# ElijahHyndman/PAPTeam_OpticalFlow

Measured on AMD Instinct MI355X. Metric: Mpix/s per frame-pair (fixed SOR iters) at 1920x1080; max-abs d(u,v) vs ref, higher is better.
Workload: dtype f64

## Files before the change

include/papof.h:

```cpp
#ifndef PAPOF_H
#define PAPOF_H

#include <stddef.h>

#ifdef __cplusplus
extern "C" {
#endif

#define PAPOF_VERSION 115

enum {
    PAPOF_OK = 0,
    PAPOF_EINVAL = -1,
    PAPOF_ENODEVICE = -2,
    PAPOF_ENOMEM = -3,
    PAPOF_EDEVICE = -4,
    PAPOF_ETIMEOUT = -5
};

enum {
    PAPOF_SOR_EXACT = 0,
    PAPOF_SOR_REDBLACK = 1,
    PAPOF_SOR_JACOBI = 2
};
// ... 443 lines not shown

int papof_deblur_tensor(papof_handle* h, int n_frames, int height, int width, int c, const papof_tensor* frames,
                        const papof_tensor* flow_fw, const papof_tensor* flow_bw, int n_samples, const double* offsets,
                        const double* weights, int radius, int iters, int use_check, double alpha1, double alpha2,
                        const papof_tensor* out, const papof_tensor* support, void* workspace, long long workspace_bytes,
                        void* stream);
long long papof_deblur_workspace(int n_frames, int height, int width, int c, int radius);

enum { PAPOF_ROWS_MAX_KNOTS = 4096 };
int papof_warp_rows_tensor(papof_handle* h, int n_frames, int height, int width, int c, const papof_tensor* frames,
                           const papof_tensor* matrices, int n_knots, int iters, const papof_tensor* out,
                           const papof_tensor* valid, void* stream);

int papof_last_host_times(papof_handle* h, double out[3]);

int papof_test_sor_strips(papof_handle* h, int height, int width, int n_sor, int split_band, int reps, int delay_us,
                          long long* mismatches, int* bands);

int papof_test_poison(papof_handle* h, unsigned long long pattern, size_t* bytes);

#ifdef __cplusplus
}
#endif
#endif
```

papteam_opticalflow_amd/capi.py:

```python
import ctypes
import os

import numpy as np

_HERE = os.path.dirname(os.path.abspath(__file__))
LIB_PATH = os.path.join(_HERE, "csrc", "libpapof.so")

SOR_EXACT, SOR_REDBLACK, SOR_JACOBI = 0, 1, 2
N_TIMERS = 10

_D = ctypes.POINTER(ctypes.c_double)
_I = ctypes.POINTER(ctypes.c_int)
c_int, c_double, c_void_p = ctypes.c_int, ctypes.c_double, ctypes.c_void_p


class Params(ctypes.Structure):
    _fields_ = [("alpha", c_double), ("ratio", c_double), ("n_outer", c_int), ("n_outer_per_level", c_int),
                ("n_inner", c_int), ("n_sor", c_int), ("n_sor_per_level", c_int), ("omega", c_double),
                ("sor_mode", c_int), ("phase_timing", c_int), ("interpolation", c_int), ("noise_model", c_int)]


DTYPE_U8, DTYPE_F32, DTYPE_F64 = 0, 1, 2
DTYPE_U16 = 3
MOTION_SIMILARITY, MOTION_AFFINE = 0, 1
# ... 17 lines not shown

SYMBOLS = [
    "papof_version", "papof_default_params", "papof_strerror", "papof_last_error", "papof_timing_key",
    "papof_device_count", "papof_create", "papof_destroy", "papof_coarse2fine_flow", "papof_flow",
    "papof_flow_device", "papof_dev_alloc", "papof_dev_free", "papof_dev_upload", "papof_dev_download",
    "papof_stream", "papof_stage_pyramid", "papof_stage_gaussian", "papof_stage_resize_ratio",
    "papof_stage_resize_wh", "papof_stage_im2feature", "papof_stage_warpFL", "papof_stage_getDxs",
    "papof_stage_linear_system", "papof_stage_laplacian", "papof_stage_sor", "papof_stage_smoothflow",
    "papof_stage_bicubic_warp", "papof_bench_sor", "papof_flow_u8", "papof_flow_device_u8", "papof_seq_reset",
    "papof_seq_push", "papof_seq_push_u8", "papof_seq_push_device", "papof_tiles_grid", "papof_tiles_rect",
    "papof_tiles_halo_message", "papof_tiles_unique_id", "papof_tiles_create", "papof_tiles_create_local",
    "papof_tiles_flow_device", "papof_tiles_stats", "papof_tiles_destroy", "papof_flow_quantize16",
    "papof_flow_dequantize16", "papof_flow_to_bgr", "papof_set_stream_overlap", "papof_sor_plan", "papof_last_sor_stats", "papof_test_sor_strips",
    "papof_pyramid_levels_for_min_width", "papof_stage_smoothflow_ex", "papof_stage_est_gaussian_mixture",
    "papof_stage_bicubic_warp_ex", "papof_tiles_comm_info", "papof_host_alloc", "papof_host_free",
    "papof_last_sor_solves", "papof_bands_plan", "papof_lap_guard_stats", "papof_last_host_times",
    "papof_flow_batch", "papof_flow_batch_u8", "papof_batch_stats", "papof_flow_batch_tensor", "papof_flow_batch_tensor_fb",
    "papof_fb_check_tensor", "papof_track_tensor", "papof_interp_tensor", "papof_flow_batch_tensor_init",
    "papof_flow_batch_tensor_fb_init", "papof_motion_fit_tensor", "papof_motion_workspace", "papof_warp_affine_tensor",
    "papof_temporal_filter_tensor", "papof_fill_holes_tensor", "papof_fill_workspace", "papof_propagate_tensor",
    "papof_temporal_consistency_tensor", "papof_consistency_workspace", "papof_splat_tensor", "papof_splat_workspace",
    "papof_interp_splat_tensor", "papof_refine_flow_tensor", "papof_refine_workspace", "papof_refine_tables",
    "papof_super_resolve_tensor", "papof_sr_workspace", "papof_match_tensor", "papof_match_workspace",
    "papof_match_hier_tensor", "papof_match_hier_workspace", "papof_match_recentre_tensor", "papof_match_recentre_workspace",
    "papof_match_densify_tensor", "papof_motion_blur_tensor", "papof_decimate_tensor", "papof_upsample_flow_tensor",
    "papof_upsample_tables", "papof_mosaic_tensor", "papof_mosaic_blend_tensor", "papof_mosaic_overlap_tensor", "papof_sor_tiny_shape",
    "papof_homography_workspace", "papof_homography_fit_tensor", "papof_warp_projective_tensor",
    "papof_mosaic_projective_tensor", "papof_mosaic_overlap_projective_tensor",
    "papof_mosaic_ray_tensor", "papof_mosaic_overlap_ray_tensor",
    "papof_bundle_workspace", "papof_bundle_sums_tensor",
    "papof_mesh_workspace", "papof_mesh_motion_tensor", "papof_warp_mesh_tensor",
# ... 84 lines not shown
    L.papof_stage_smoothflow_ex.argtypes = [c_void_p, _D, _D, _D, _D, _D, c_int, c_int, c_int, c_double, c_int, c_int,
                                            c_int, c_double, c_int, c_int, c_int, _D]
    L.papof_stage_est_gaussian_mixture.argtypes = [c_void_p, _D, _D, c_int, c_int, c_int, _D]
    L.papof_stage_bicubic_warp_ex.argtypes = [c_void_p, _D, _D, _D, _D, c_int, c_int, c_int, c_int, _D]
    L.papof_pyramid_levels_for_min_width.argtypes = [c_int, c_double, c_int, ctypes.POINTER(c_int)]
    L.papof_sor_tiny_shape.argtypes = [c_int, c_int, ctypes.POINTER(c_int), ctypes.POINTER(c_int)]
    L.papof_host_alloc.argtypes = [ctypes.c_size_t, ctypes.POINTER(c_void_p)]
    L.papof_host_free.argtypes = [c_void_p]
    L.papof_sor_plan.argtypes = [c_void_p, c_int, c_int, c_int, c_int, ctypes.POINTER(c_int), ctypes.POINTER(c_int)]
    L.papof_last_sor_stats.argtypes = [c_void_p, ctypes.POINTER(c_int), ctypes.POINTER(ctypes.c_double)]
    L.papof_last_sor_solves.argtypes = [c_void_p, c_int, ctypes.POINTER(c_int), ctypes.POINTER(c_int),
                                        ctypes.POINTER(ctypes.c_double)]
    L.papof_lap_guard_stats.argtypes = [c_void_p, ctypes.POINTER(c_int)]
    L.papof_last_host_times.argtypes = [c_void_p, ctypes.POINTER(c_double)]
    L.papof_batch_stats.argtypes = [c_void_p, ctypes.POINTER(ctypes.c_longlong)]
    for fn in (L.papof_flow_batch, L.papof_flow_batch_u8):
        fn.argtypes = [c_void_p, c_int, c_int, c_void_p, c_int, c_int, c_int, c_int, c_void_p, c_void_p, c_void_p, c_void_p, _D]
        fn.restype = c_int
    _T = ctypes.POINTER(PapofTensor)
    L.papof_flow_batch_tensor.argtypes = [c_void_p, c_int, c_int, _T, _T, c_int, c_int, c_int, c_int, PP, _T, _T, c_void_p, _D]
    L.papof_flow_batch_tensor.restype = c_int
    L.papof_flow_batch_tensor_fb.argtypes = [c_void_p, c_int, c_int, _T, _T, c_int, c_int, c_int, c_int, PP, _T, _T, _T, _T, _T,
                                             c_double, c_double, c_void_p, _D]
    L.papof_flow_batch_tensor_fb.restype = c_int
    L.papof_flow_batch_tensor_init.argtypes = [c_void_p, c_int, c_int, _T, _T, c_int, c_int, c_int, c_int, PP, _T, _T, _T,
                                               c_void_p, _D]
    L.papof_flow_batch_tensor_init.restype = c_int
    L.papof_flow_batch_tensor_fb_init.argtypes = [c_void_p, c_int, c_int, _T, _T, c_int, c_int, c_int, c_int, PP, _T, _T, _T,
                                                  _T, _T, _T, _T, c_double, c_double, c_void_p, _D]
    L.papof_flow_batch_tensor_fb_init.restype = c_int
# ... 587 lines not shown
        t = np.zeros(N_TIMERS)
        PP = ctypes.c_void_p * len(fr)
        fp = PP(*[f.ctypes.data for f in fr])
        OP = ctypes.c_void_p * n_pairs
        ox, oy, ow = (OP(*[o[i].ctypes.data for o in out]) for i in range(3))
        pp = ctypes.byref(params) if params is not None else None
        fn = self.L.papof_flow_batch_u8 if u8 else self.L.papof_flow_batch
        _chk(fn(self.h, n_pairs, 1 if sequence else 0, fp, h, w, c, int(levels), pp, ox, oy, ow, _p(t)), "papof_flow_batch")
        return out, t

    def batch_stats(self):
        out = (ctypes.c_longlong * 4)()
        _chk(self.L.papof_batch_stats(self.h, out), "papof_batch_stats")
        return dict(chains=out[0], chain_pairs=out[1], singles=out[2], reruns=out[3])

    def last_host_times(self):
        out = (c_double * 3)()
        _chk(self.L.papof_last_host_times(self.h, out), "papof_last_host_times")
        return out[0], out[1]

    def lap_guard_stats(self):
        out = (c_int * 4)()
        _chk(self.L.papof_lap_guard_stats(self.h, out), "papof_lap_guard_stats")
        return dict(reruns=out[0], exact_calls=out[1], exact_next=bool(out[2]), guard_on=bool(out[3]))

    def test_sor_strips(self, h, w, n_sor, split_band, reps=3, delay_us=0):
        mm, nb = ctypes.c_longlong(0), c_int(0)
        _chk(self.L.papof_test_sor_strips(self.h, h, w, n_sor, split_band, reps, delay_us, ctypes.byref(mm),
                                          ctypes.byref(nb)), "papof_test_sor_strips")
        return mm.value, nb.value

    def test_poison(self, pattern=0x7FF8DEAD7FF8DEAD):
        n = ctypes.c_size_t(0)
        _chk(self.L.papof_test_poison(self.h, pattern, ctypes.byref(n)), "papof_test_poison")
# ... 179 lines not shown
```

papteam_opticalflow_amd/csrc/api.hip:

```cpp
#include <algorithm>
#include <chrono>
#include <cmath>
#include <cstdio>
#include <cstdlib>
#include <cstring>
#include <mutex>
#include <random>
#include <thread>

#include "common.h"
#include "flow_internal.h"

namespace papof {

namespace {
thread_local std::string g_last_error;
}

void set_last_error(const char* what, hipError_t e, const char* file, int line) {
    char buf[512];
    std::snprintf(buf, sizeof buf, "%s failed: %s (%s:%d)", what, hipGetErrorString(e), file, line);
    g_last_error = buf;
}
const char* last_error() { return g_last_error.c_str(); }
// ... 302 lines not shown

struct LevelSolve {
    SolveBuffers& B;
    const double *f1 = nullptr, *f2 = nullptr;
    double* warp = nullptr;
    int H = 0, W = 0, fc = 0;
    double alpha = 0, omega = 0;
    int n_outer = 0, n_inner = 0, n_sor = 0, mode = PAPOF_SOR_EXACT;
    const double* im1s_ready = nullptr;
    bool final_warp = true;
    const SolveCounters* counters = nullptr;
    double *out_u = nullptr, *out_v = nullptr;
    bool fold_warp = false;
    LapGuard* lg = nullptr;
    int level = 0;
};

static int marked_solve(papof_handle* h, PhaseClock& clk, unsigned* prog, SorPlanes& SP, const LevelSolve& s) {
    h->sor_mark = [](void* c, int on) {
        static_cast<PhaseClock*>(c)->phase(on ? PAPOF_T_PHASE5_SOR : PAPOF_T_PHASE6_UPDATE);
    };
    h->sor_mark_ctx = &clk;
    h->sor_prog_next = prog;
    const int rc = sor_solve(h, SP, s.H, s.W, s.alpha, s.omega, s.n_sor, s.mode);
    h->sor_prog_next = nullptr;
    h->sor_mark = nullptr;
    h->sor_mark_ctx = nullptr;
    return rc;
}

int smooth_flow(papof_handle* h, const LevelSolve& s, PhaseClock& clk, double*& u, double*& v, double*& ua, double*& va) {
    SolveBuffers& B = s.B;
    const Taps g = smooth5_taps();
    int solve_idx = 0;
    const bool tiny = s.mode == PAPOF_SOR_EXACT && B.sp_tiny.phi && sor_tiny_fits(h, s.H, s.W, s.n_sor);
    SorPlanes& SP = tiny ? B.sp_tiny : B.sp;
    const double* im1s = s.im1s_ready;
    if (!im1s) {
        clk.phase(PAPOF_T_PHASE1_GENERATE);
        PAPOF_TRY(filter_hv(h, s.f1, B.im1s, B.tmp, s.H, s.W, s.fc, g, g));
        im1s = B.im1s;
    }
    const char* const fused_sw = std::getenv("PAPOF_FUSED_SYSTEM");
    const bool fused_env = !(fused_sw && fused_sw[0] == '0');
    const bool fused_system = fused_env && s.fold_warp && s.n_inner == 1 && !B.gm && (s.fc == 5 || s.fc == 3) &&
                              !(s.lg && s.lg->guard()) && !(s.lg && s.lg->on && lap_one_block_level(s.H, s.W));
    for (int count = 0; count < s.n_outer; count++) {
        clk.phase(fused_system ? kTimerFused : (int)PAPOF_T_PHASE1_GENERATE);
        if (fused_system)
            PAPOF_TRY(flow_system(h, s.f1, s.f2, u, v, im1s, s.H, s.W, s.fc, s.alpha, s.omega, SP,
                                  s.lg && count > 0 ? s.lg->wit(s.lg->slot - 1) : nullptr));
        else if (s.fold_warp)
            PAPOF_TRY(warp_smooth_blend(h, s.f1, s.f2, u, v, im1s, B.blend, B.imdt, s.H, s.W, s.fc,
                                        s.lg && count > 0 && !B.gm ? s.lg->wit(s.lg->slot - 1) : nullptr,
                                        B.phi));
        else
            PAPOF_TRY(smooth_hv_blend(h, s.warp, im1s, B.blend, B.imdt, s.H, s.W, s.fc));
        for (int hh = 0; hh < s.n_inner; hh++) {
            const SorPlanes* prev = hh == 0 ? nullptr : &SP;
            if ((count == 0 && !s.fold_warp) || hh > 0) {
                clk.phase(PAPOF_T_PHASE2_DERIVATIVES);
                PAPOF_TRY(compute_phi(h, u, v, prev, B.phi, s.H, s.W));
            }
            if (!fused_system) clk.phase(PAPOF_T_PHASE4_LINEARSYSTEM);
            if (!fused_system)
                PAPOF_TRY(assemble_system(h, B.blend, B.imdt, B.phi, u, v, s.H, s.W, s.fc, s.alpha, s.omega, SP, nullptr, nullptr,
                                          prev, nullptr, B.gm, s.lg ? s.lg->guard() : nullptr));
            PAPOF_TRY(marked_solve(h, clk, s.counters ? s.counters->solve(h, s.level, (size_t)solve_idx) : nullptr, SP, s));
            solve_idx++;
        }
        double* const phi_next = count + 1 < s.n_outer && !s.fold_warp ? B.phi : nullptr;
        const bool rewarp = !s.fold_warp && !B.bgx && (s.final_warp || count + 1 < s.n_outer || B.gm);
        const bool wit_later = s.fold_warp && count + 1 < s.n_outer;
        const bool wit_small = s.fold_warp && !wit_later && lap_one_block_level(s.H, s.W);
        unsigned* const wit = s.lg && !B.gm && !B.bgx && !wit_later && !wit_small ? s.lg->wit(s.lg->slot) : nullptr;
        const bool to_caller = s.out_u && s.out_v && count + 1 == s.n_outer;
        PAPOF_TRY(update_warp_phi(h, SP, u, v, to_caller ? s.out_u : ua, to_caller ? s.out_v : va, s.f1, s.f2, s.warp, phi_next,
                                  s.H, s.W, s.fc, rewarp, 0, -1, wit));
        if (to_caller) {
            u = s.out_u;
            v = s.out_v;
        } else {
            std::swap(u, ua);
            std::swap(v, va);
        }
        if (B.bgx)
            PAPOF_TRY(bicubic_warp(h, s.f1, s.f2, B.bgx, B.bgy, B.bgxy, u, v, s.warp, s.H, s.W, s.fc, nullptr, true, true));
        if (s.lg && s.lg->on && !B.gm && wit_small && s.lg->wit(s.lg->slot))
            PAPOF_TRY(lap_small_check(h, s.f1, s.f2, u, v, s.H, s.W, s.fc, s.lg->wit(s.lg->slot)));
        if (s.lg && s.lg->on && !B.gm) {
            s.lg->slot_level.push_back(s.level);
            s.lg->slot_channels.push_back(s.fc);
            s.lg->slot++;
            if (s.lg->exact) {
// ... 43 lines not shown
    LapGuard* lg;
    const papof_tensor* init;
    CallPlan cp;
    int slot1 = 0;
    double *tmp_a = nullptr, *tmp_b = nullptr;
    std::vector<double*> F1, F2, S1;
    double *prep_tmp = nullptr, *warp = nullptr;
    double *u = nullptr, *v = nullptr, *u2 = nullptr, *v2 = nullptr;
    SolveBuffers B;
    bool exact = false;
    SolveCounters counters;
    bool overlap = false;
    bool hostio = false;
    hipStream_t main_stream = nullptr, prep = nullptr;
    PhaseClock clk, pclk, total;
};

static void keep_seq(const FlowPass& S, int slot) {
    S.h->seq = {.valid = true, .h = S.H, .w = S.W, .c = S.C, .levels = S.cp.levels, .slot = slot, .ratio = S.cp.ratio,
                .arena_base = S.h->arena.base};
}

static void start_clocks(FlowPass& S) {
    papof_handle* h = S.h;
    S.clk = S.pclk = S.total = PhaseClock{h, true};
    S.clk.only_sor = S.pclk.only_sor = (!h->phase_events && S.P.phase_timing == 0) || S.P.phase_timing == 2;
    h->sor_launches = 0;
    h->sor_log.clear();
    S.clk.stamps = true;
    h->stamps_used = 0;
    h->next_stamp = nullptr;
    h->stamp_stream = h->stream;
    S.total.phase(PAPOF_T_TOTAL);
}

static int carve_pyramids(FlowPass& S) {
    Arena& A = S.h->arena;
    for (Level& l : S.cp.L) {
        double* slot[2];
        slot[0] = A.f64((size_t)l.w * l.h * S.C);
        slot[1] = A.f64((size_t)l.w * l.h * S.C);
        l.p1 = slot[S.slot1];
        l.p2 = slot[S.slot1 ^ 1];
// ... 139 lines not shown
    S.v = S.u + np;
    S.v2 = S.u2 + np;
    if (B.bgx) PAPOF_TRY(central3_planes(h, f2, B.bgx, B.bgy, B.bgxy, lh, lw, fc));
    if (coarsest && !S.init) return PAPOF_OK;
    if (B.bgx)
        PAPOF_TRY(bicubic_warp(h, f1, f2, B.bgx, B.bgy, B.bgxy, S.u, S.v, S.warp, lh, lw, fc, nullptr, true, false));
    else if (!fold_warp)
        PAPOF_TRY(warp_bilinear(h, f1, f2, S.u, S.v, S.warp, lh, lw, fc));
    return PAPOF_OK;
}

static int solve_levels(FlowPass& S) {
    papof_handle* h = S.h;
    const CallPlan& cp = S.cp;
    LapGuard* const lg = S.lg;
    if (lg && lg->guard())
        PAPOF_HIP(hipMemcpyAsync(lg->lap, h->lap_init_dev, 8 * sizeof(double), hipMemcpyDeviceToDevice, S.main_stream));
    int pw = 0, ph = 0;
    for (int k = cp.levels - 1; k >= 0; k--) {
        const int lw = cp.L[k].w, lh = cp.L[k].h;
        S.clk.phase(-1);
        if (S.overlap) PAPOF_HIP(hipStreamWaitEvent(S.main_stream, h->sync_events[k], 0));
        S.clk.phase(PAPOF_T_ALLOCATION);
        const bool tiny_k = S.exact && sor_tiny_fits(h, lh, lw, cp.n_sor[k]);
        if (!tiny_k) PAPOF_TRY(sor_bind(h, S.B.sp, lh, lw, cp.n_sor[k]));
        const LevelSolve s{.B = S.B, .f1 = S.F1[k], .f2 = S.F2[k], .warp = S.warp, .H = lh, .W = lw, .fc = cp.fc,
                           .alpha = S.P.alpha, .omega = S.P.omega, .n_outer = cp.n_outer[k], .n_inner = S.P.n_inner,
                           .n_sor = cp.n_sor[k], .mode = S.P.sor_mode, .im1s_ready = S.S1[k], .final_warp = false,
                           .counters = S.exact ? &S.counters : nullptr, .out_u = k == 0 ? S.d_vx : nullptr,
                           .out_v = k == 0 ? S.d_vy : nullptr, .fold_warp = !S.B.bgx && !S.B.gm, .lg = lg, .level = k};
        PAPOF_TRY(enter_level(S, k, pw, ph, s.fold_warp));
        if (!tiny_k) PAPOF_TRY(sor_reset_planes(h, S.B.sp));
        PAPOF_TRY(smooth_flow(h, s, S.clk, S.u, S.v, S.u2, S.v2));
        pw = lw;
        ph = lh;
    }
    return PAPOF_OK;
}

static int final_warp(FlowPass& S) {
    papof_handle* h = S.h;
    papof_handle::HostIO& io = h->hostio;
    const int H = S.H, W = S.W, C = S.C;
    const size_t np0 = (size_t)H * W;
    const Level& l0 = S.cp.L[0];
    S.clk.phase(PAPOF_T_POSTPROCESSING);
    if (S.hostio && io.early_out && S.u == S.d_vx && S.v == S.d_vy) {
// ... 49 lines not shown
    }
    {
        const double f = tm[kTimerFused];
        tm[PAPOF_T_PHASE1_GENERATE] += 0.51 * f;
        tm[PAPOF_T_PHASE2_DERIVATIVES] += 0.02 * f;
        tm[PAPOF_T_PHASE3_PSIDATA] += 0.14 * f;
        tm[PAPOF_T_PHASE4_LINEARSYSTEM] += f - 0.51 * f - 0.02 * f - 0.14 * f;
    }
}

int flow_pass(papof_handle* h, const FrameIn& fa, const FrameIn& fb, SeqOp op, int H, int W, int C, int levels,
              const papof_params& P, double* d_vx, double* d_vy, double* d_warp, double* timing, LapGuard* lg,
              const papof_tensor* init = nullptr) {
    const double t_entry = wall();
    FlowPass S{h, fa, fb, op, H, W, C, P, d_vx, d_vy, d_warp, lg, init};
    PAPOF_TRY(call_plan(H, W, C, levels, P, S.cp));
    const size_t need = arena_bytes_for(H, W, C, levels, S.cp.n_sor_max, P.ratio);
    if (op == kSeqNext && !seq_matches(h, H, W, C, levels, S.cp.ratio, need)) {
        g_last_error = "sequence push does not continue the primed sequence (shape, levels, ratio or arena changed)";
        return PAPOF_EINVAL;
    }
    S.slot1 = op == kSeqNext ? h->seq.slot : 0;
    h->seq.valid = false;
    PAPOF_TRY(ensure_arena(h, need));
    h->arena.off = 0;
    h->arena.overflow = false;
    h->events_used = 0;
    double tm[PAPOF_N_TIMERS + 1];
    std::memset(tm, 0, sizeof tm);
    start_clocks(S);
// ... 974 lines not shown
}

int papof_lap_guard_stats(papof_handle* h, int out[4]) {
    if (!h || !out) return PAPOF_EINVAL;
    out[0] = h->lap_reruns;
    out[1] = h->lap_exact_calls;
    out[2] = h->lap_exact ? 1 : 0;
    out[3] = h->lap_guard ? 1 : 0;
    return PAPOF_OK;
}

int papof_last_host_times(papof_handle* h, double out[3]) {
    if (!h || !out) return PAPOF_EINVAL;
    out[0] = h->host_enqueue_sec;
    out[1] = h->host_wait_sec;
    out[2] = 0.0;
    return PAPOF_OK;
}

int papof_last_sor_solves(papof_handle* h, int cap, int* n, int* info, double* sec) {
    if (!h || !n) return PAPOF_EINVAL;
    *n = (int)h->sor_log.size();
    for (int i = 0; i < *n && i < cap; i++) {
        const papof_handle::SorSolveLog& e = h->sor_log[i];
        if (info) {
            int* o = info + (size_t)i * 6;
            o[0] = e.H;
            o[1] = e.W;
            o[2] = e.n_sor;
            o[3] = e.kind;
            o[4] = e.depth;
// ... 229 lines not shown
```

papteam_opticalflow_amd/csrc/common.h:

```cpp
#pragma once
#include <cstdlib>

#include <hip/hip_runtime.h>

#include <algorithm>
#include <cmath>
#include <cstddef>
#include <cstdint>
#include <initializer_list>
#include <string>
#include <vector>

#include "../../include/papof.h"

namespace papof {

constexpr int kLanes = 64;
constexpr int kMaxFsize = 8;

struct Rect {
    int x0, y0, x1, y1;
    __host__ __device__ bool empty() const { return x1 <= x0 || y1 <= y0; }
    __host__ __device__ int w() const { return x1 - x0; }
    __host__ __device__ int h() const { return y1 - y0; }
// ... 155 lines not shown
    hipEvent_t entry_event = nullptr;
    unsigned* init_flag_dev = nullptr;
    bool use_dpp = false;
    int sor_depth = 0;
    unsigned long long* sor_dbg = nullptr;
    void (*sor_mark)(void*, int) = nullptr;
    void* sor_mark_ctx = nullptr;
    int sor_fuse = 0;
    int sor_group = 0;
    int rb_depth = 0;
    int rb_shape = 0;
    int sor_tiny = 1;
    int sor_resident = 0;
    int sor_skip_dead = 1;
    unsigned* sor_prog_next = nullptr;
    int sor_launches = 0;
    struct SorSolveLog {
        int H, W, n_sor, kind, depth, launches;
        double sec;
    };
    std::vector<SorSolveLog> sor_log;
    hipStream_t prep_stream = nullptr;
    unsigned* lap_flags_dev = nullptr;
    unsigned* lap_flags_host = nullptr;
    double* lap_dev = nullptr;
    double* lap_init_dev = nullptr;
    double* lap_scratch_dev = nullptr;
    bool lap_guard = true;
    bool lap_exact = false;
    unsigned lap_epoch = 0;
    int lap_reruns = 0, lap_exact_calls = 0;
    long long batch_chains = 0, batch_chain_pairs = 0, batch_singles = 0, batch_reruns = 0;
    double host_enqueue_sec = 0.0, host_wait_sec = 0.0;
    struct HostIO {
        bool active = false;
        const void *im1 = nullptr, *im2 = nullptr;
        size_t nb_in = 0;
        double *vx = nullptr, *vy = nullptr, *warp = nullptr;
        size_t nb_flow = 0, nb_img = 0;
        bool early_out = false;
        bool out_issued = false;
    } hostio;
    hipStream_t copy_stream = nullptr;
    std::vector<hipEvent_t> copy_events;
    std::vector<hipEvent_t> sync_events;
    bool overlap_prep = true;
    unsigned long long* stamps_dev = nullptr;
// ... 72 lines not shown
                   int W, int planes, const Rect* rc = nullptr);
int smooth_hv_blend(papof_handle* h, const double* warp, const double* im1s, double* blend, double* imdt, int H,
                    int W, int planes, int row0 = 0, int row1 = -1);
int warp_smooth_blend(papof_handle* h, const double* im1, const double* im2, const double* u, const double* v,
                      const double* im1s, double* blend, double* imdt, int H, int W, int planes, unsigned* wit = nullptr,
                      double* phi_out = nullptr);
int compute_phi(papof_handle* h, const double* u, const double* v, const SorPlanes* prev, double* phi, int H, int W,
                const Rect* rc = nullptr);
int assemble_system(papof_handle* h, const double* blend, const double* imdt, const double* phi, const double* u,
                    const double* v, int H, int W, int planes, double alpha, double omega, const SorPlanes& out,
                    double* opt_imdx2, double* opt_imdy2, const SorPlanes* prev, const Rect* rc = nullptr,
                    const double* gm = nullptr, const double* lap = nullptr);
int flow_system(papof_handle* h, const double* im1, const double* im2, const double* u, const double* v, const double* im1s,
                int H, int W, int planes, double alpha, double omega, const SorPlanes& out, unsigned* wit = nullptr,
                int row0 = 0, int row1 = -1,
                int batch = 1, const BatchK* bk = nullptr);
int lap_scratch_doubles();
int lap_rows_check(papof_handle* h, const double* im1, const double* im2, const double* u, const double* v, int H, int W,
                   int C, int r0, int r1, unsigned* wit, unsigned* val, unsigned mark);
bool lap_one_block_level(int H, int W);
int lap_small_check(papof_handle* h, const double* im1, const double* im2, const double* u, const double* v, int H, int W,
                    int C, unsigned* wit, int batch = 1, const BatchK* bk = nullptr);
int est_laplacian_noise(papof_handle* h, const double* im1, const double* im2, const double* u, const double* v, int H,
                        int W, int C, double* lap, double* scratch);
int gm_scratch_doubles();
int est_gaussian_mixture(papof_handle* h, const double* im1, const double* im2, int H, int W, int C, double* gm,
                         double* scratch);
int laplacian(papof_handle* h, const double* in, const double* weight, double* out, int H, int W);
int bicubic_warp(papof_handle* h, const double* im1, const double* im2, const double* gx, const double* gy,
                 const double* gxy, const double* vx, const double* vy, double* out_hwc, int H, int W, int C,
                 const Rect* rc = nullptr, bool planar_out = false, bool clamp = true, int batch = 1, const BatchK* bk = nullptr);
// ... 33 lines not shown
};
int sor_solve_bands(papof_handle* h, const SorPlanes& sp, int H, int W, double alpha, double omega, int n_sor,
                    unsigned* prog, int b0, int b1, const SorSplit* split = nullptr);
int sor_bind_plain(papof_handle* h, SorPlanes& sp, int H, int W, int n_sor);
constexpr size_t kTinyMaxCells = 8192;
bool sor_tiny_fits(const papof_handle* h, int H, int W, int n_sor);
bool sor_tiny_shape(int H, int W, int* cells_per_tile, int* waves);
int sor_alloc_tiny_planes(Arena& A, size_t cells, SorPlanes& sp);
size_t sor_counters_words(int H, int W, int n_sor);
int sor_counters_ensure(papof_handle* h, size_t words);
unsigned* sor_counters_clear(papof_handle* h, size_t offset_words, size_t words);
int sor_alloc_planes(Arena& A, int H, int W, int mode, int n_sor_cap, SorPlanes& sp);
int sor_bind(papof_handle* h, SorPlanes& sp, int H, int W, int n_sor);
int sor_group_size(const papof_handle* h, int H, int W, int n_sor);
int sor_reset_planes(papof_handle* h, const SorPlanes& sp);
int sor_reset_planes_batch(papof_handle* h, const SorPlanes& sp, int batch, size_t stride);
int sor_probe_dpp(papof_handle* h);

}
```

papteam_opticalflow_amd/csrc/kernels.hip:

```cpp
#include "common.h"
#include "sampler.h"

#include <cmath>
#include <type_traits>

namespace papof {

namespace {

constexpr int BX = 64, BY = 4;

constexpr int tiles_of(int n, int t) { return (n + t - 1) / t; }
inline dim3 grid2d(int W, int H, int planes = 1) { return dim3(tiles_of(W, BX), tiles_of(H, BY), planes); }
inline Rect region(const Rect* rc, int W, int H) { return rc ? *rc : Rect{0, 0, W, H}; }
inline dim3 grid2d(const Rect& r, int planes = 1) { return grid2d(r.x1 - r.x0, r.y1 - r.y0, planes); }

__device__ __forceinline__ void stamp_now(unsigned long long* s) {
    if (s && (blockIdx.x | blockIdx.y | blockIdx.z | threadIdx.x | threadIdx.y) == 0u) *s = __builtin_amdgcn_s_memrealtime();
}
__global__ void k_stamp(unsigned long long* s) { stamp_now(s); }

__host__ __device__ __forceinline__ int clampi(int x, int n) {
    x = x < 0 ? 0 : x;
    return x > n - 1 ? n - 1 : x;
// ... 989 lines not shown
    double* q[6];
};
typedef double tap_pair __attribute__((ext_vector_type(2), aligned(8)));
__device__ __forceinline__ double plane_ld(const double* plane, unsigned byte_off) {
    return *reinterpret_cast<const double*>(reinterpret_cast<const char*>(plane) + byte_off);
}
__device__ __forceinline__ tap_pair plane_ld2(const double* plane, unsigned byte_off) {
    return *reinterpret_cast<const tap_pair*>(reinterpret_cast<const char*>(plane) + byte_off);
}
template <int PLANES, bool SKEW, bool BATCH = false, bool W1 = false>
__global__ __launch_bounds__(256, 1) void k_flow_system(const double* __restrict__ im1, const double* __restrict__ im2,
                                                     const double* __restrict__ u, const double* __restrict__ v,
                                                     const double* __restrict__ im1s, int H, int W, double alpha,
                                                     double omega, SkewIdx sk, SixPlanes out, Taps g, Taps d,
                                                     unsigned long long* stamp, unsigned* __restrict__ wit, double wit_thr,
                                                     unsigned mark, int row0, int row1, BatchK bk) {
    if (BATCH) {
        const size_t p = blockIdx.y;
        im1s += batch_frames(bk, p, im1, im2);
        u += p * bk.uv;
        v += p * bk.uv;
        if (wit != nullptr) wit += p * bk.wit;
#pragma unroll
        for (int q = 0; q < 6; q++) out.q[q] += p * bk.sp;
    }
    constexpr int NT = kFT * kFT, HWc = kFT + 2 * kFH;
    __shared__ double raw[kFW][HWc + 1];
    __shared__ double hs[kFW][kFT + 4 + 1];
    __shared__ double bl[kFT + 4][kFT + 4 + 1];
    __shared__ double it[kFT][kFT + 1];
    __shared__ double ph[kFT + 1][kFT + 1 + 1];
    __shared__ double stage[6][kFT][kFT + 1];
    stamp_now(stamp);
    const int ntx = (W + kFT - 1) / kFT, ntiles = ntx * ((row1 - row0 + kFT - 1) / kFT), per = (ntiles + 7) >> 3;
    const int vt = (int)(blockIdx.x & 7u) * per + (int)(blockIdx.x >> 3);
    if ((int)(blockIdx.x >> 3) >= per || vt >= ntiles) return;
    const int tby = vt / ntx, tbx = vt - tby * ntx;
    const int ib = row0 + tby * kFT, j0 = tbx * kFT, tid = threadIdx.x;
    const size_t np = (size_t)H * W;
    const int vy0 = max(0, row0 - kFH), vy1 = min(H, row1 + kFH);
    const bool interior = ib >= vy0 + kFH && ib + kFT <= row1 && ib + kFT + kFH <= vy1 && j0 >= kFH && j0 + kFT + kFH <= W;
    constexpr int kPer = (kFW * HWc + NT - 1) / NT;
    static_assert(kFW * HWc == 2 * NT + 64 && NT + 16 < kFW * HWc, "the three slots of the warp");
    const int lane = tid & 63, wave = __builtin_amdgcn_readfirstlane(tid >> 6);
    constexpr bool w1 = W1;
    unsigned t_o[kPer], t_b0[kPer], t_b1[kPer];
    int t_ra[kPer];
// ... 18 lines not shown
                    r++;
                }
                if (cc >= HWc) {
                    cc -= HWc;
                    r++;
                }
            }
            const int i = ib - kFH + r, j = j0 - kFH + cc;
            t_ra[q] = r * (HWc + 1) + cc;
            t_in[q] = i >= vy0 && i < vy1 && j >= 0 && j < W;
            const int o = t_in[q] ? i * W + j : 0;
            t_o[q] = (unsigned)o * 8u;
            double x = 0.0, y = 0.0;
            t_out[q] = false;
            if (t_in[q]) {
                y = i + v[o];
                x = j + u[o];
                t_out[q] = leaves_image(x, y, W, H);
                if (t_out[q]) {
                    x = j;
                    y = i;
                }
            }
            const int x0 = (int)x, y0 = (int)y, y1 = min(y0 + 1, H - 1);
            const int xb = w1 ? 0 : min(x0, W - 2);
            t_hi[q] = x0 == W - 1;
            t_b0[q] = (unsigned)(y0 * W + xb) * 8u;
            t_b1[q] = (unsigned)(y1 * W + xb) * 8u;
            t_dx[q] = x - x0;
            t_dy[q] = y - y0;
        }
    }
    const bool wout = __ballot(t_out[0] || t_out[1] || t_out[2]) != 0ull;
    for (int c = tid; c < (kFT + 1) * (kFT + 1); c += NT) {
        const int r = c / (kFT + 1), cc = c - r * (kFT + 1);
        const int i = ib - 1 + r, j = j0 - 1 + cc;
        if (i < 0 || i >= min(H, row1) || j < 0 || j >= W) continue;
        const size_t o = (size_t)i * W + j;
        const double uc = u[o], vc = v[o];
        double ur = 0.0, vr = 0.0, ud = 0.0, vd = 0.0;
        if (j < W - 1) {
            ur = u[o + 1];
            vr = v[o + 1];
        }
        if (i < H - 1) {
            ud = u[o + W];
            vd = v[o + W];
        }
        ph[r][cc] = phi_value(uc, vc, ur, vr, ud, vd, j < W - 1, i < H - 1);
    }
    const int orow = tid / kFT, ocol = tid - orow * kFT;
    const int oi = ib + orow, oj = j0 + ocol;
    const bool own = oi < row1 && oj < W;
    PsiTerms s;
    const bool sampler = wit != nullptr && tid < 64 &&
                         lap_samples_here(ntiles, tbx, tby);
    constexpr int kP3 = ((kFT + 4) * (kFT + 4) + NT - 1) / NT;
    int s_r[kP3], s_c[kP3];
    unsigned s_o[kP3];
    static_assert(kP3 == 2 && kFW * (kFT + 4) / 2 <= NT && (kFT + 4) * (kFT + 4) / 2 <= NT, "two outputs per thread");
    const int h_r = tid / ((kFT + 4) / 2), h_c = 2 * (tid - h_r * ((kFT + 4) / 2));
    {
// ... 123 lines not shown
                for (int l = -2; l <= 2; l++) gx += bl[orow + 2][clampi(oj + l, W) - (j0 - 2)] * d.t[l + 2];
#pragma unroll
                for (int l = -2; l <= 2; l++) gy += bl[clampi(oi + l, H) - (ib - 2)][ocol + 2] * d.t[l + 2];
            }
            const double gt = it[orow][ocol];
            double t = gt;
            t *= t;
            s.add(psi_value(t), gx, gy, gt, PLANES == 1);
        }
    }
    if (own) {
        s.mean(PLANES);
        const size_t o = (size_t)oi * W + oj;
        const Nbrs n = nbrs_at(oi, oj, H, W);
        const PhiAround p{ph[orow + 1][ocol + 1], n.left ? ph[orow + 1][ocol] : 0.0, n.up ? ph[orow][ocol + 1] : 0.0};
        const SystemCell c = system_cell<true>(s, p, cross_at<true>(u, o, W, n), cross_at<true>(v, o, W, n), n, alpha, omega);
        if (SKEW) {
            stage_cell(stage, orow, ocol, c);
        } else {
            out.q[0][o] = c.phi;
            out.q[1][o] = c.xy;
            out.q[2][o] = c.a1;
            out.q[3][o] = c.a2;
            out.q[4][o] = c.b1;
            out.q[5][o] = c.b2;
        }
    }
    if (!SKEW) return;
    __syncthreads();
    store_skew_tile(stage, tid, ib, j0, row1, W, sk, reinterpret_cast<double2s*>(out.q[0]),
                    reinterpret_cast<double2s*>(out.q[2]), reinterpret_cast<double2s*>(out.q[4]));
// ... 711 lines not shown
        hipLaunchKernelGGL(kern, dim3(tiles_of(W, kTileJ), tiles_of(r.y1 - r.y0, kAsmRows)),
                           dim3(256), 0, h->stream, blend, imdt, phi, u, v, H, W, planes, alpha, omega, skew_idx(out),
                           (double2s*)out.phi, (double2s*)out.a1, (double2s*)out.b1, opt_imdx2, opt_imdy2,
                           deriv5_taps(), I, take_stamp(h), r.y0, r.y1);
    } else {
        hipLaunchKernelGGL(k_assemble, grid2d(r), dim3(BX, BY), 0, h->stream, blend, imdt, phi, u, v, H, W, planes,
                           alpha, omega, out.phi, out.xy, out.a1, out.a2, out.b1, out.b2, opt_imdx2, opt_imdy2,
                           deriv5_taps(), I, r, take_stamp(h));
    }
    LAUNCH_CHECK();
    return PAPOF_OK;
}

int flow_system(papof_handle* h, const double* im1, const double* im2, const double* u, const double* v, const double* im1s,
                int H, int W, int planes, double alpha, double omega, const SorPlanes& out, unsigned* wit, int row0, int row1,
                int batch, const BatchK* bk) {
    if (planes != 5 && planes != 3) return PAPOF_EINVAL;
    if ((unsigned long long)H * (unsigned long long)W > (1ull << 29)) return PAPOF_EINVAL;
    int rc;
    if (!rows_of(row0, row1, H, rc)) return rc;
    const dim3 grid(xcd_grid(tiles_of(W, kFT), tiles_of(row1 - row0, kFT)), batch);
    const SixPlanes six{{out.phi, out.xy, out.a1, out.a2, out.b1, out.b2}};
    const auto kern = with_flags([](auto five, auto skew, auto batched, auto one_column) {
        return &k_flow_system<five.value ? 5 : 3, skew.value, batched.value, one_column.value>;
    }, planes == 5, out.skew, batch > 1, W == 1);
    hipLaunchKernelGGL(kern, grid, dim3(kFT * kFT), 0, h->stream, im1, im2, u, v, im1s, H, W, alpha, omega,
                       out.skew ? skew_idx(out) : kNoSkew, six, smooth5_taps(), deriv5_taps(),
                       take_stamp(h), wit, lap_wit_threshold(H, W), h->lap_epoch, row0, row1, bk ? *bk : kNoBatch);
    LAUNCH_CHECK();
    return PAPOF_OK;
}

int laplacian(papof_handle* h, const double* in, const double* weight, double* out, int H, int W) {
    hipLaunchKernelGGL(k_laplacian, grid2d(W, H), dim3(BX, BY), 0, h->stream, in, weight, out, H, W);
    LAUNCH_CHECK();
    return PAPOF_OK;
}

int update_warp_phi(papof_handle* h, const SorPlanes& sp, const double* u, const double* v, double* u_out, double* v_out,
                    const double* im1, const double* im2, double* warp, double* phi_out, int H, int W, int planes,
                    bool do_warp, int row0, int row1, unsigned* wit, int batch, const BatchK* bk) {
    if (batch > 1 && (warp || phi_out || do_warp)) return PAPOF_EINVAL;
    if (u == u_out || v == v_out) return PAPOF_EINVAL;
    int rc;
    if (!rows_of(row0, row1, H, rc)) return rc;
    const dim3 grid(xcd_grid(tiles_of(W, BX), tiles_of(row1 - row0, BY)), batch);
    const auto kern = with_flags([](auto skew, auto batched) { return &k_update_warp_phi<skew.value, batched.value>; },
                                 sp.skew, batch > 1);
    hipLaunchKernelGGL(kern, grid, dim3(BX, BY), 0, h->stream, sp.du, sp.dv, sp.skew ? skew_idx(sp) : kNoSkew, u, v, u_out,
                       v_out, im1, im2, warp, phi_out, H, W, planes, do_warp ? 1 : 0, take_stamp(h), row0, row1, wit,
                       lap_wit_threshold(H, W), h->lap_epoch, bk ? *bk : kNoBatch);
    LAUNCH_CHECK();
    return PAPOF_OK;
}

int update_flow(papof_handle* h, const SorPlanes& sp, double* u, double* v, int H, int W, const Rect& r) {
    if (sp.skew) return PAPOF_EINVAL;
    if (r.empty()) return PAPOF_OK;
    hipLaunchKernelGGL(k_update_warp, grid2d(r), dim3(BX, BY), 0, h->stream, sp.du, sp.dv, u, v, nullptr, nullptr, nullptr,
                       H, W, 0, r, 0, take_stamp(h));
    LAUNCH_CHECK();
    return PAPOF_OK;
}

int flow_quantize16(papof_handle* h, const double* vx, const double* vy, unsigned short* q, size_t n) {
    if (!n) return PAPOF_OK;
// ... 265 lines not shown
```

papteam_opticalflow_amd/csrc/sor.hip:

```cpp
#include <algorithm>
#include <cstdio>
#include <cstdlib>
#include <cstring>
#include <type_traits>

#include "common.h"

namespace papof {

namespace {

#ifndef PAPOF_V_DM6
#define PAPOF_V_DM6 4
#endif
#ifndef PAPOF_V_DM8
#define PAPOF_V_DM8 5
#endif
#ifndef PAPOF_V_FDM6
#define PAPOF_V_FDM6 3
#endif
#ifndef PAPOF_V_FDM8
#define PAPOF_V_FDM8 4
#endif
#ifndef PAPOF_V_FMIDPOLL
// ... 1541 lines not shown
    } else if (mode == PAPOF_SOR_REDBLACK || mode == PAPOF_SOR_JACOBI) {
        const BlockedPlan bp = blocked_plan(h, mode, H, W, mode == PAPOF_SOR_REDBLACK ? 2 * n_sor : n_sor);
        nl = bp.n_launch;
        d = bp.q * (bp.base + (bp.rem ? 1 : 0));
    } else {
        return PAPOF_EINVAL;
    }
    if (launches) *launches = nl;
    if (depth) *depth = d;
    return PAPOF_OK;
}

int sor_solve(papof_handle* h, const SorPlanes& sp, int H, int W, double alpha, double omega, int n_sor, int mode,
              const SorBatch* bt) {
    const double nalpha = -alpha, om1 = 1 - omega;
    if (n_sor <= 0) return PAPOF_EINVAL;
    const int batch = bt ? bt->n : 1;
    if (batch < 1 || (bt && mode != PAPOF_SOR_EXACT)) return PAPOF_EINVAL;
    const auto mark = [&](int on) {
        if (h->sor_mark) h->sor_mark(h->sor_mark_ctx, on);
    };
    const auto log_solve = [&](int kind, int depth, int launches) {
        if (h->sor_log.size() >= 4096) h->sor_log.clear();
        h->sor_log.push_back(papof_handle::SorSolveLog{H, W, n_sor, kind, depth, launches, 0.0});
    };
    if (mode == PAPOF_SOR_EXACT && !sp.skew) {
        mark(1);
        PAPOF_TRY(sor_tiny_solve(h, sp, H, W, alpha, omega, n_sor, batch, bt ? bt->tiny : 0));
        mark(0);
        log_solve(6, 0, 1);
// ... 25 lines not shown
        } else {
            const size_t nbytes = (size_t)sd.nb * n_sor * kProgStride * sizeof(unsigned);
            PAPOF_HIP(hipMemsetAsync(prog, 0, nbytes, h->stream));
        }
        ExactArgs A = exact_args(h, sp, sd, H, W, alpha, omega, n_sor, prog);
        if (bt) {
            A.bs_coef = bt->coef;
            A.bs_d = bt->d;
            A.bs_prog = bt->prog;
        } else {
            A.dbg = h->sor_dbg;
        }
        if (std::getenv("PAPOF_SOR_INJECT_ABORT")) PAPOF_HIP(hipMemsetAsync(h->sync_words, 1, sizeof(unsigned), h->stream));
        if (bt) {
            PAPOF_TRY(fill_pairs(h, sp.du, bt->d * sizeof(double), sd.nd * 16, batch));
        } else {
            PAPOF_HIP(hipMemsetAsync(sp.du, 0, (sd.nd + sd.nh) * 16, h->stream));
        }
        mark(1);
        if (sd.group > 1) {
            GroupArgs Ga;
            Ga.phi = sp.phi;
            Ga.a1 = sp.a1;
            Ga.b1 = sp.b1;
            Ga.du = sp.du;
            Ga.prog = prog;
            Ga.abort = h->sync_words;
            Ga.nb = sd.nb;
            Ga.ns = sd.ns;
            Ga.hp = sd.hp;
            Ga.npos = sd.npos;
            Ga.qt = sd.qt;
// ... 164 lines not shown

static size_t plane_pitch(const SkewDims& sd) { return 2 * (((size_t)sd.n + kLanes + 63) / 64 * 64); }
static void pack_planes(SorPlanes& sp) {
    const size_t pitch = plane_pitch(sp.sd);
    sp.xy = sp.phi + 1;
    sp.a1 = sp.phi + pitch;
    sp.a2 = sp.a1 + 1;
    sp.b1 = sp.a1 + pitch;
    sp.b2 = sp.b1 + 1;
}
int sor_reset_planes(papof_handle* h, const SorPlanes& sp) {
    if (!sp.skew) return PAPOF_OK;
    PAPOF_HIP(hipMemsetAsync(sp.phi, 0, 3 * plane_pitch(sp.sd) * sizeof(double), h->stream));
    return PAPOF_OK;
}

int sor_reset_planes_batch(papof_handle* h, const SorPlanes& sp, int batch, size_t stride) {
    if (!sp.skew) return PAPOF_OK;
    return fill_pairs(h, sp.phi, stride * sizeof(double), 3 * plane_pitch(sp.sd) * sizeof(double), batch);
}

int sor_group_size(const papof_handle* h, int H, int W, int n_sor) {
    if (!h || !h->use_dpp || n_sor < 2) return 1;
    int g = h->sor_group;
    if (g == 0 && h->sor_fuse == 2) return 1;
    if (g == 0) {
        const int nb = skew_dims(H, W, n_sor).nb;
        g = ((nb <= 2 && n_sor >= 36) || (nb == 3 && n_sor >= 50)) ? 4 : 1;
    }
    if (g >= 4) return 4;
// ... 111 lines not shown
```

Before: 218.2.

## Carry SOR increments into fused flow system, skipping separate update_warp_phi pass

In the fused-system outer loop, the flow_system kernel now adds the previous SOR increments (du,dv) to u,v itself. It writes the updated flow out and caches it in shared memory for the phi and cross computations. This skips the separate update_warp_phi launch between outer iterations and replaces the per-solve du memset with one clear per level, relying on the SOR solve to overwrite du fully. It adds shared memory per block and a swap of u/ua buffers, and correctness depends on the du buffer invariant holding across solves.

After: 223.4, median of 6. +2.4%, better.

```diff
diff --git a/include/papof.h b/include/papof.h
--- a/include/papof.h
+++ b/include/papof.h
@@ -481,6 +481,8 @@
 
 int papof_last_host_times(papof_handle* h, double out[3]);
 
+int papof_last_chain_stats(papof_handle* h, long long out[4]);
+
 int papof_test_sor_strips(papof_handle* h, int height, int width, int n_sor, int split_band, int reps, int delay_us,
                           long long* mismatches, int* bands);
 
diff --git a/papteam_opticalflow_amd/capi.py b/papteam_opticalflow_amd/capi.py
--- a/papteam_opticalflow_amd/capi.py
+++ b/papteam_opticalflow_amd/capi.py
@@ -55,7 +55,7 @@
     "papof_flow_dequantize16", "papof_flow_to_bgr", "papof_set_stream_overlap", "papof_sor_plan", "papof_last_sor_stats", "papof_test_sor_strips",
     "papof_pyramid_levels_for_min_width", "papof_stage_smoothflow_ex", "papof_stage_est_gaussian_mixture",
     "papof_stage_bicubic_warp_ex", "papof_tiles_comm_info", "papof_host_alloc", "papof_host_free",
-    "papof_last_sor_solves", "papof_bands_plan", "papof_lap_guard_stats", "papof_last_host_times",
+    "papof_last_sor_solves", "papof_bands_plan", "papof_lap_guard_stats", "papof_last_host_times", "papof_last_chain_stats",
     "papof_flow_batch", "papof_flow_batch_u8", "papof_batch_stats", "papof_flow_batch_tensor", "papof_flow_batch_tensor_fb",
     "papof_fb_check_tensor", "papof_track_tensor", "papof_interp_tensor", "papof_flow_batch_tensor_init",
     "papof_flow_batch_tensor_fb_init", "papof_motion_fit_tensor", "papof_motion_workspace", "papof_warp_affine_tensor",
@@ -170,6 +170,8 @@
     L.papof_lap_guard_stats.argtypes = [c_void_p, ctypes.POINTER(c_int)]
     L.papof_last_host_times.argtypes = [c_void_p, ctypes.POINTER(c_double)]
     L.papof_batch_stats.argtypes = [c_void_p, ctypes.POINTER(ctypes.c_longlong)]
+    if hasattr(L, "papof_last_chain_stats"):
+        L.papof_last_chain_stats.argtypes = [c_void_p, ctypes.POINTER(ctypes.c_longlong)]
     for fn in (L.papof_flow_batch, L.papof_flow_batch_u8):
         fn.argtypes = [c_void_p, c_int, c_int, c_void_p, c_int, c_int, c_int, c_int, c_void_p, c_void_p, c_void_p, c_void_p, _D]
         fn.restype = c_int
@@ -787,10 +789,15 @@
         _chk(self.L.papof_batch_stats(self.h, out), "papof_batch_stats")
         return dict(chains=out[0], chain_pairs=out[1], singles=out[2], reruns=out[3])
 
-    def last_host_times(self):
+    def last_host_times(self, first_solve=False):
         out = (c_double * 3)()
         _chk(self.L.papof_last_host_times(self.h, out), "papof_last_host_times")
-        return out[0], out[1]
+        return (out[0], out[1], out[2]) if first_solve else (out[0], out[1])
+
+    def last_chain_stats(self):
+        out = (ctypes.c_longlong * 4)()
+        _chk(self.L.papof_last_chain_stats(self.h, out), "papof_last_chain_stats")
+        return dict(flow_systems=out[0], carried=out[1], updates=out[2], clears=out[3])
 
     def lap_guard_stats(self):
         out = (c_int * 4)()
diff --git a/papteam_opticalflow_amd/csrc/api.hip b/papteam_opticalflow_amd/csrc/api.hip
--- a/papteam_opticalflow_amd/csrc/api.hip
+++ b/papteam_opticalflow_amd/csrc/api.hip
@@ -340,6 +340,7 @@
     bool fold_warp = false;
     LapGuard* lg = nullptr;
     int level = 0;
+    bool dudv_cleared = false;
 };
 
 static int marked_solve(papof_handle* h, PhaseClock& clk, unsigned* prog, SorPlanes& SP, const LevelSolve& s) {
@@ -348,6 +349,7 @@
     };
     h->sor_mark_ctx = &clk;
     h->sor_prog_next = prog;
+    h->sor_dudv_cleared = s.dudv_cleared && &SP == &s.B.sp;
     const int rc = sor_solve(h, SP, s.H, s.W, s.alpha, s.omega, s.n_sor, s.mode);
     h->sor_prog_next = nullptr;
     h->sor_mark = nullptr;
@@ -371,12 +373,19 @@
     const bool fused_env = !(fused_sw && fused_sw[0] == '0');
     const bool fused_system = fused_env && s.fold_warp && s.n_inner == 1 && !B.gm && (s.fc == 5 || s.fc == 3) &&
                               !(s.lg && s.lg->guard()) && !(s.lg && s.lg->on && lap_one_block_level(s.H, s.W));
+    bool carried = false;
     for (int count = 0; count < s.n_outer; count++) {
         clk.phase(fused_system ? kTimerFused : (int)PAPOF_T_PHASE1_GENERATE);
-        if (fused_system)
+        if (fused_system) {
             PAPOF_TRY(flow_system(h, s.f1, s.f2, u, v, im1s, s.H, s.W, s.fc, s.alpha, s.omega, SP,
-                                  s.lg && count > 0 ? s.lg->wit(s.lg->slot - 1) : nullptr));
-        else if (s.fold_warp)
+                                  s.lg && count > 0 ? s.lg->wit(s.lg->slot - 1) : nullptr, 0, -1, 1, nullptr,
+                                  carried ? &SP : nullptr, carried ? ua : nullptr, carried ? va : nullptr));
+            if (carried) {
+                std::swap(u, ua);
+                std::swap(v, va);
+                carried = false;
+            }
+        } else if (s.fold_warp)
             PAPOF_TRY(warp_smooth_blend(h, s.f1, s.f2, u, v, im1s, B.blend, B.imdt, s.H, s.W, s.fc,
                                         s.lg && count > 0 && !B.gm ? s.lg->wit(s.lg->slot - 1) : nullptr,
                                         B.phi));
@@ -401,9 +410,12 @@
         const bool wit_small = s.fold_warp && !wit_later && lap_one_block_level(s.H, s.W);
         unsigned* const wit = s.lg && !B.gm && !B.bgx && !wit_later && !wit_small ? s.lg->wit(s.lg->slot) : nullptr;
         const bool to_caller = s.out_u && s.out_v && count + 1 == s.n_outer;
-        PAPOF_TRY(update_warp_phi(h, SP, u, v, to_caller ? s.out_u : ua, to_caller ? s.out_v : va, s.f1, s.f2, s.warp, phi_next,
-                                  s.H, s.W, s.fc, rewarp, 0, -1, wit));
-        if (to_caller) {
+        carried = fused_system && count + 1 < s.n_outer;
+        if (!carried)
+            PAPOF_TRY(update_warp_phi(h, SP, u, v, to_caller ? s.out_u : ua, to_caller ? s.out_v : va, s.f1, s.f2, s.warp,
+                                      phi_next, s.H, s.W, s.fc, rewarp, 0, -1, wit));
+        if (carried) {
+        } else if (to_caller) {
             u = s.out_u;
             v = s.out_v;
         } else {
@@ -477,6 +489,7 @@
     bool hostio = false;
     hipStream_t main_stream = nullptr, prep = nullptr;
     PhaseClock clk, pclk, total;
+    double t_entry = 0.0;
 };
 
 static void keep_seq(const FlowPass& S, int slot) {
@@ -490,6 +503,7 @@
     S.clk.only_sor = S.pclk.only_sor = (!h->phase_events && S.P.phase_timing == 0) || S.P.phase_timing == 2;
     h->sor_launches = 0;
     h->sor_log.clear();
+    std::fill(h->chain_stats, h->chain_stats + 4, 0LL);
     S.clk.stamps = true;
     h->stamps_used = 0;
     h->next_stamp = nullptr;
@@ -659,6 +673,7 @@
     papof_handle* h = S.h;
     const CallPlan& cp = S.cp;
     LapGuard* const lg = S.lg;
+    h->host_first_solve_sec = wall() - S.t_entry;
     if (lg && lg->guard())
         PAPOF_HIP(hipMemcpyAsync(lg->lap, h->lap_init_dev, 8 * sizeof(double), hipMemcpyDeviceToDevice, S.main_stream));
     int pw = 0, ph = 0;
@@ -669,13 +684,14 @@
         S.clk.phase(PAPOF_T_ALLOCATION);
         const bool tiny_k = S.exact && sor_tiny_fits(h, lh, lw, cp.n_sor[k]);
         if (!tiny_k) PAPOF_TRY(sor_bind(h, S.B.sp, lh, lw, cp.n_sor[k]));
-        const LevelSolve s{.B = S.B, .f1 = S.F1[k], .f2 = S.F2[k], .warp = S.warp, .H = lh, .W = lw, .fc = cp.fc,
-                           .alpha = S.P.alpha, .omega = S.P.omega, .n_outer = cp.n_outer[k], .n_inner = S.P.n_inner,
-                           .n_sor = cp.n_sor[k], .mode = S.P.sor_mode, .im1s_ready = S.S1[k], .final_warp = false,
-                           .counters = S.exact ? &S.counters : nullptr, .out_u = k == 0 ? S.d_vx : nullptr,
-                           .out_v = k == 0 ? S.d_vy : nullptr, .fold_warp = !S.B.bgx && !S.B.gm, .lg = lg, .level = k};
+        LevelSolve s{.B = S.B, .f1 = S.F1[k], .f2 = S.F2[k], .warp = S.warp, .H = lh, .W = lw, .fc = cp.fc,
+                     .alpha = S.P.alpha, .omega = S.P.omega, .n_outer = cp.n_outer[k], .n_inner = S.P.n_inner,
+                     .n_sor = cp.n_sor[k], .mode = S.P.sor_mode, .im1s_ready = S.S1[k], .final_warp = false,
+                     .counters = S.exact ? &S.counters : nullptr, .out_u = k == 0 ? S.d_vx : nullptr,
+                     .out_v = k == 0 ? S.d_vy : nullptr, .fold_warp = !S.B.bgx && !S.B.gm, .lg = lg, .level = k};
         PAPOF_TRY(enter_level(S, k, pw, ph, s.fold_warp));
         if (!tiny_k) PAPOF_TRY(sor_reset_planes(h, S.B.sp));
+        if (!tiny_k && S.exact) PAPOF_TRY(sor_reset_dudv(h, S.B.sp, &s.dudv_cleared));
         PAPOF_TRY(smooth_flow(h, s, S.clk, S.u, S.v, S.u2, S.v2));
         pw = lw;
         ph = lh;
@@ -755,6 +771,7 @@
               const papof_tensor* init = nullptr) {
     const double t_entry = wall();
     FlowPass S{h, fa, fb, op, H, W, C, P, d_vx, d_vy, d_warp, lg, init};
+    S.t_entry = t_entry;
     PAPOF_TRY(call_plan(H, W, C, levels, P, S.cp));
     const size_t need = arena_bytes_for(H, W, C, levels, S.cp.n_sor_max, P.ratio);
     if (op == kSeqNext && !seq_matches(h, H, W, C, levels, S.cp.ratio, need)) {
@@ -1759,7 +1776,13 @@
     if (!h || !out) return PAPOF_EINVAL;
     out[0] = h->host_enqueue_sec;
     out[1] = h->host_wait_sec;
-    out[2] = 0.0;
+    out[2] = h->host_first_solve_sec;
+    return PAPOF_OK;
+}
+
+int papof_last_chain_stats(papof_handle* h, long long out[4]) {
+    if (!h || !out) return PAPOF_EINVAL;
+    std::copy(h->chain_stats, h->chain_stats + 4, out);
     return PAPOF_OK;
 }
 
diff --git a/papteam_opticalflow_amd/csrc/common.h b/papteam_opticalflow_amd/csrc/common.h
--- a/papteam_opticalflow_amd/csrc/common.h
+++ b/papteam_opticalflow_amd/csrc/common.h
@@ -193,6 +193,8 @@
     int sor_resident = 0;
     int sor_skip_dead = 1;
     unsigned* sor_prog_next = nullptr;
+    long long chain_stats[4] = {0, 0, 0, 0};
+    bool sor_dudv_cleared = false;
     int sor_launches = 0;
     struct SorSolveLog {
         int H, W, n_sor, kind, depth, launches;
@@ -210,6 +212,7 @@
     unsigned lap_epoch = 0;
     int lap_reruns = 0, lap_exact_calls = 0;
     long long batch_chains = 0, batch_chain_pairs = 0, batch_singles = 0, batch_reruns = 0;
+    double host_first_solve_sec = 0.0;
     double host_enqueue_sec = 0.0, host_wait_sec = 0.0;
     struct HostIO {
         bool active = false;
@@ -312,7 +315,8 @@
 int flow_system(papof_handle* h, const double* im1, const double* im2, const double* u, const double* v, const double* im1s,
                 int H, int W, int planes, double alpha, double omega, const SorPlanes& out, unsigned* wit = nullptr,
                 int row0 = 0, int row1 = -1,
-                int batch = 1, const BatchK* bk = nullptr);
+                int batch = 1, const BatchK* bk = nullptr,
+                const SorPlanes* inc = nullptr, double* u_out = nullptr, double* v_out = nullptr);
 int lap_scratch_doubles();
 int lap_rows_check(papof_handle* h, const double* im1, const double* im2, const double* u, const double* v, int H, int W,
                    int C, int r0, int r1, unsigned* wit, unsigned* val, unsigned mark);
@@ -376,6 +380,7 @@
 int sor_bind(papof_handle* h, SorPlanes& sp, int H, int W, int n_sor);
 int sor_group_size(const papof_handle* h, int H, int W, int n_sor);
 int sor_reset_planes(papof_handle* h, const SorPlanes& sp);
+int sor_reset_dudv(papof_handle* h, const SorPlanes& sp, bool* done);
 int sor_reset_planes_batch(papof_handle* h, const SorPlanes& sp, int batch, size_t stride);
 int sor_probe_dpp(papof_handle* h);
 
diff --git a/papteam_opticalflow_amd/csrc/kernels.hip b/papteam_opticalflow_amd/csrc/kernels.hip
--- a/papteam_opticalflow_amd/csrc/kernels.hip
+++ b/papteam_opticalflow_amd/csrc/kernels.hip
@@ -1027,7 +1027,9 @@
                                                      const double* __restrict__ im1s, int H, int W, double alpha,
                                                      double omega, SkewIdx sk, SixPlanes out, Taps g, Taps d,
                                                      unsigned long long* stamp, unsigned* __restrict__ wit, double wit_thr,
-                                                     unsigned mark, int row0, int row1, BatchK bk) {
+                                                     unsigned mark, int row0, int row1, BatchK bk,
+                                                     const double* __restrict__ sdu, const double* __restrict__ sdv,
+                                                     double* __restrict__ u_out, double* __restrict__ v_out) {
     if (BATCH) {
         const size_t p = blockIdx.y;
         im1s += batch_frames(bk, p, im1, im2);
@@ -1044,6 +1046,7 @@
     __shared__ double it[kFT][kFT + 1];
     __shared__ double ph[kFT + 1][kFT + 1 + 1];
     __shared__ double stage[6][kFT][kFT + 1];
+    __shared__ double fu[kFW][HWc + 1], fv[kFW][HWc + 1];
     stamp_now(stamp);
     const int ntx = (W + kFT - 1) / kFT, ntiles = ntx * ((row1 - row0 + kFT - 1) / kFT), per = (ntiles + 7) >> 3;
     const int vt = (int)(blockIdx.x & 7u) * per + (int)(blockIdx.x >> 3);
@@ -1092,8 +1095,24 @@
             double x = 0.0, y = 0.0;
             t_out[q] = false;
             if (t_in[q]) {
-                y = i + v[o];
-                x = j + u[o];
+                double pu = u[o], pv = v[o];
+                if (sdu != nullptr) {
+                    double a, b;
+                    if (SKEW) {
+                        const double2s c = reinterpret_cast<const double2s*>(sdu)[dudv_cell(i, j, sk)];
+                        a = c.x;
+                        b = c.y;
+                    } else {
+                        a = sdu[o];
+                        b = sdv[o];
+                    }
+                    pu += a;
+                    pv += b;
+                }
+                (&fu[0][0])[t_ra[q]] = pu;
+                (&fv[0][0])[t_ra[q]] = pv;
+                y = i + pv;
+                x = j + pu;
                 t_out[q] = leaves_image(x, y, W, H);
                 if (t_out[q]) {
                     x = j;
@@ -1110,20 +1129,21 @@
         }
     }
     const bool wout = __ballot(t_out[0] || t_out[1] || t_out[2]) != 0ull;
+    __syncthreads();
     for (int c = tid; c < (kFT + 1) * (kFT + 1); c += NT) {
         const int r = c / (kFT + 1), cc = c - r * (kFT + 1);
         const int i = ib - 1 + r, j = j0 - 1 + cc;
         if (i < 0 || i >= min(H, row1) || j < 0 || j >= W) continue;
-        const size_t o = (size_t)i * W + j;
-        const double uc = u[o], vc = v[o];
+        const double *const pu = &fu[r + kFH - 1][cc + kFH - 1], *const pv = &fv[r + kFH - 1][cc + kFH - 1];
+        const double uc = pu[0], vc = pv[0];
         double ur = 0.0, vr = 0.0, ud = 0.0, vd = 0.0;
         if (j < W - 1) {
-            ur = u[o + 1];
-            vr = v[o + 1];
+            ur = pu[1];
+            vr = pv[1];
         }
         if (i < H - 1) {
-            ud = u[o + W];
-            vd = v[o + W];
+            ud = pu[HWc + 1];
+            vd = pv[HWc + 1];
         }
         ph[r][cc] = phi_value(uc, vc, ur, vr, ud, vd, j < W - 1, i < H - 1);
     }
@@ -1277,7 +1297,15 @@
         const size_t o = (size_t)oi * W + oj;
         const Nbrs n = nbrs_at(oi, oj, H, W);
         const PhiAround p{ph[orow + 1][ocol + 1], n.left ? ph[orow + 1][ocol] : 0.0, n.up ? ph[orow][ocol + 1] : 0.0};
-        const SystemCell c = system_cell<true>(s, p, cross_at<true>(u, o, W, n), cross_at<true>(v, o, W, n), n, alpha, omega);
+        const auto cross = [&](const double* c) {
+            return Cross{c[0], c[n.left ? -1 : 0], c[n.right ? 1 : 0], c[n.up ? -(HWc + 1) : 0], c[n.down ? HWc + 1 : 0]};
+        };
+        const Cross cu = cross(&fu[orow + kFH][ocol + kFH]), cv = cross(&fv[orow + kFH][ocol + kFH]);
+        if (u_out != nullptr) {
+            u_out[o] = cu.c;
+            v_out[o] = cv.c;
+        }
+        const SystemCell c = system_cell<true>(s, p, cu, cv, n, alpha, omega);
         if (SKEW) {
             stage_cell(stage, orow, ocol, c);
         } else {
@@ -2019,8 +2047,12 @@
 
 int flow_system(papof_handle* h, const double* im1, const double* im2, const double* u, const double* v, const double* im1s,
                 int H, int W, int planes, double alpha, double omega, const SorPlanes& out, unsigned* wit, int row0, int row1,
-                int batch, const BatchK* bk) {
+                int batch, const BatchK* bk, const SorPlanes* inc, double* u_out, double* v_out) {
     if (planes != 5 && planes != 3) return PAPOF_EINVAL;
+    if (inc && (batch > 1 || row0 != 0 || (row1 >= 0 && row1 != H) || inc->skew != out.skew || !inc->du || !u_out || !v_out ||
+                u_out == u || v_out == v))
+        return PAPOF_EINVAL;
+    if (!inc && (u_out || v_out)) return PAPOF_EINVAL;
     if ((unsigned long long)H * (unsigned long long)W > (1ull << 29)) return PAPOF_EINVAL;
     int rc;
     if (!rows_of(row0, row1, H, rc)) return rc;
@@ -2031,7 +2063,10 @@
     }, planes == 5, out.skew, batch > 1, W == 1);
     hipLaunchKernelGGL(kern, grid, dim3(kFT * kFT), 0, h->stream, im1, im2, u, v, im1s, H, W, alpha, omega,
                        out.skew ? skew_idx(out) : kNoSkew, six, smooth5_taps(), deriv5_taps(),
-                       take_stamp(h), wit, lap_wit_threshold(H, W), h->lap_epoch, row0, row1, bk ? *bk : kNoBatch);
+                       take_stamp(h), wit, lap_wit_threshold(H, W), h->lap_epoch, row0, row1, bk ? *bk : kNoBatch,
+                       inc ? inc->du : nullptr, inc ? inc->dv : nullptr, u_out, v_out);
+    h->chain_stats[0]++;
+    h->chain_stats[1] += inc != nullptr;
     LAUNCH_CHECK();
     return PAPOF_OK;
 }
@@ -2055,6 +2090,7 @@
     hipLaunchKernelGGL(kern, grid, dim3(BX, BY), 0, h->stream, sp.du, sp.dv, sp.skew ? skew_idx(sp) : kNoSkew, u, v, u_out,
                        v_out, im1, im2, warp, phi_out, H, W, planes, do_warp ? 1 : 0, take_stamp(h), row0, row1, wit,
                        lap_wit_threshold(H, W), h->lap_epoch, bk ? *bk : kNoBatch);
+    h->chain_stats[2]++;
     LAUNCH_CHECK();
     return PAPOF_OK;
 }
diff --git a/papteam_opticalflow_amd/csrc/sor.hip b/papteam_opticalflow_amd/csrc/sor.hip
--- a/papteam_opticalflow_amd/csrc/sor.hip
+++ b/papteam_opticalflow_amd/csrc/sor.hip
@@ -1579,6 +1579,8 @@
 int sor_solve(papof_handle* h, const SorPlanes& sp, int H, int W, double alpha, double omega, int n_sor, int mode,
               const SorBatch* bt) {
     const double nalpha = -alpha, om1 = 1 - omega;
+    const bool dudv_cleared = h->sor_dudv_cleared;
+    h->sor_dudv_cleared = false;
     if (n_sor <= 0) return PAPOF_EINVAL;
     const int batch = bt ? bt->n : 1;
     if (batch < 1 || (bt && mode != PAPOF_SOR_EXACT)) return PAPOF_EINVAL;
@@ -1634,8 +1636,9 @@
         if (std::getenv("PAPOF_SOR_INJECT_ABORT")) PAPOF_HIP(hipMemsetAsync(h->sync_words, 1, sizeof(unsigned), h->stream));
         if (bt) {
             PAPOF_TRY(fill_pairs(h, sp.du, bt->d * sizeof(double), sd.nd * 16, batch));
-        } else {
+        } else if (!(dudv_cleared && sd.group == 1)) {
             PAPOF_HIP(hipMemsetAsync(sp.du, 0, (sd.nd + sd.nh) * 16, h->stream));
+            h->chain_stats[3]++;
         }
         mark(1);
         if (sd.group > 1) {
@@ -1830,6 +1833,13 @@
     PAPOF_HIP(hipMemsetAsync(sp.phi, 0, 3 * plane_pitch(sp.sd) * sizeof(double), h->stream));
     return PAPOF_OK;
 }
+int sor_reset_dudv(papof_handle* h, const SorPlanes& sp, bool* done) {
+    *done = false;
+    if (!sp.skew || sp.sd.group != 1) return PAPOF_OK;
+    PAPOF_HIP(hipMemsetAsync(sp.du, 0, sp.sd.nd * 16, h->stream));
+    *done = true;
+    return PAPOF_OK;
+}
 
 int sor_reset_planes_batch(papof_handle* h, const SorPlanes& sp, int batch, size_t stride) {
     if (!sp.skew) return PAPOF_OK;
```
